# TimoStoff/event_utils

Measured on AMD Instinct MI355X. Metric: Mevents/s (voxel 5-bin 640x480), higher is better.
Workload: dtype f32

## Files before the change

### event_utils_amd/csrc/evk_image2.hip

```cpp
#include "evk_part2.h"
#include "evk_splat.h"

namespace evk {

struct SrcImgF32 {
    static constexpr int G = 4, XYW = 8, TPW = 4;
    const float *x, *y, *w;
    float clipx, clipy;
    float *img;
    int h, wd;
    template <bool NT = false>
    __device__ __forceinline__ void load_xy(int64_t ev0, uint32_t gl, uint32_t *r) const {
        const uint4 a = load_col16<NT>(reinterpret_cast<const float *>(x), ev0, gl), b = load_col16<NT>(reinterpret_cast<const float *>(y), ev0, gl);
        r[0] = a.x, r[1] = a.y, r[2] = a.z, r[3] = a.w, r[4] = b.x, r[5] = b.y, r[6] = b.z, r[7] = b.w;
    }
    template <bool NT = false>
    __device__ __forceinline__ void load_tp(int64_t ev0, uint32_t gl, uint32_t *r) const {
        const uint4 a = load_col16<NT>(w, ev0, gl);
        r[0] = a.x, r[1] = a.y, r[2] = a.z, r[3] = a.w;
    }
    __device__ __forceinline__ int key_of(const uint32_t *r, int e, const TileGridG &g, uint32_t &cell) const {
        const float xf = __uint_as_float(r[e]), yf = __uint_as_float(r[4 + e]);
        const bool keep = !(xf >= clipx) & !(yf >= clipy);
        return nearest_key_cell_int(keep ? (int)xf : 0, keep ? (int)yf : 0, !keep | ((xf == xf) & (yf == yf)), g, cell);
// ... 830 lines not shown
        const int pl = i / dcells;
        __hip_atomic_store(mine + i, lds_cell(pl, i - pl * dcells), __ATOMIC_RELAXED, __HIP_MEMORY_SCOPE_AGENT);
    }
    if (!img_last_part(index, ntiles, it)) return;
    const float *parts = staging + (int64_t)it.first_item * stride;
    flush([&](int pl, int c) {
        float sum = 0.0f;
        for (uint32_t pp = 0; pp < it.nparts; ++pp)
            sum += __hip_atomic_load(parts + (int64_t)pp * stride + pl * dcells + c, __ATOMIC_RELAXED, __HIP_MEMORY_SCOPE_AGENT);
        return sum;
    });
}

static inline int img_window_cells(int tw, int th) { return (tw + 1) * (th + 1); }

static inline bool img_small(int ntiles) {
    return ntiles <= 680 || v2_part_lds(1024, 12, V2_FMT_IMGB, ntiles) > (size_t)V2_LDS_LIMIT;
}
struct ImgCall {
    TileGridG g;
    Part2 q;
    V2Layout L;
    int ntiles;
    bool small;
};
#define IMG_TS_PLANES 6
static int img_setup(ImgCall &ic, int64_t n, int h, int wd, int tile_w, int tile_h, int flags, const void *out, uint32_t *index,
                     void *scratch, int64_t scratch_bytes, uint32_t *host_report, int planes = 2, bool small_only = false) {
    const int known = EVK_VOXEL_OVERWRITE | EVK_VOXEL2_PARTITION_ONLY | EVK_VOXEL2_TILES_ONLY | EVK_VOXEL2_NO_XCD_ORDER |
                      EVK_IMAGE2_NO_FIXED;
    if (make_grid_g(ic.g, h, wd, tile_w, tile_h) != EVK_OK || !out || !index || !scratch || n <= 0 ||
        n > (int64_t)4000000000LL || (flags & ~known))
        return EVK_EINVAL;
    if (host_report && ((uintptr_t)host_report & 7u)) return EVK_EALIGN;
    ic.ntiles = ic.g.tiles_x * ic.g.tiles_y;
    if (ic.ntiles > evk_voxel2_max_tiles() || !evk_voxel2_num_tiles(h, wd, tile_w, tile_h) ||
        (tile_w + 2) * (tile_h + 1) > IMG_WIN_MAX)
        return EVK_EINVAL;
    const bool small = small_only || img_small(ic.ntiles);
    ic.small = small;
    ic.L = v2_layout(ic.ntiles, n, planes, tile_w, tile_h, small);
    if (scratch_bytes < ic.L.total) return EVK_ESCRATCH;
    if (!aligned16(scratch)) return EVK_EALIGN;
    ic.q = v2_geometry(n, ic.ntiles, small);
    return EVK_OK;
}

template <int FMT, typename C>
static void img_partition(const C &c, int64_t n, const ImgCall &ic, uint32_t *index, void *scratch, uint32_t *oob,
                          uint32_t *host_report, uint32_t seq, hipStream_t s, int t_from_events = 0) {
    char *sb = (char *)scratch;
    if constexpr (FMT == V2_FMT_IMGX || FMT == V2_FMT_IMGD) {
        launch_part<1024, 8, FMT>(c, n, ic.g, ic.ntiles, ic.q, 0.0f, 0.0f, 0.0f, t_from_events, sb + ic.L.rec, sb + ic.L.pw,
                                  (uint32_t *)(sb + ic.L.bases), (uint32_t *)(sb + ic.L.table), index, oob, host_report, seq, s);
    } else if (ic.small) {
        launch_part<1024, 8, FMT>(c, n, ic.g, ic.ntiles, ic.q, 0.0f, 0.0f, 0.0f, t_from_events, sb + ic.L.rec, sb + ic.L.pw,
                                  (uint32_t *)(sb + ic.L.bases), (uint32_t *)(sb + ic.L.table), index, oob, host_report, seq, s);
    } else {
        launch_part<1024, 12, FMT>(c, n, ic.g, ic.ntiles, ic.q, 0.0f, 0.0f, 0.0f, t_from_events, sb + ic.L.rec, sb + ic.L.pw,
                                   (uint32_t *)(sb + ic.L.bases), (uint32_t *)(sb + ic.L.table), index, oob, host_report, seq, s);
    }
}

}

using namespace evk;

// ... 194 lines not shown
```

### event_utils_amd/csrc/evk_part2.h

```cpp
#pragma once
#include <cstdio>
#include <cstring>
#include <mutex>
#include <type_traits>

#include "evk_part.h"

namespace evk {

#define V2_HDR 16
#define V2_MAX_TILES 2048
#define V2_TOTALS V2_HDR
#define V2_LIVE_PROGRESS (V2_HDR + V2_MAX_TILES)
#define V2_LIVE_STATUS (V2_LIVE_PROGRESS + 256)
#define V2_PART (V2_LIVE_STATUS + V2_MAX_TILES)
#define V2_COUNTER(T) (V2_PART + (T) + 1)
#define V2_ITEM(T) (V2_PART + 2 * (T) + 1)
#define V2_LB 10
#define EVK_VOXEL2_COUNT (1 << 20)
#define EVK_VOXEL2_COUNT2 (1 << 21)
#define V2_LOCAL_MASK ((1u << V2_LB) - 1u)
#define V2_WIDE (1u << V2_LB)
#define V2_P_MASK (~((2u << V2_LB) - 1u))
__device__ __forceinline__ void lds_barrier() { asm volatile("s_waitcnt lgkmcnt(0)\n\ts_barrier" ::: "memory"); }
// ... 372 lines not shown
                uint32_t word = (d << V2_DELTA_SHIFT) | (code << V2_CODE_SHIFT) | (kl[s2] & V2_LOCAL_MASK);
                if (__any(esc)) {
                    if (esc) {
                        const uint32_t e = atomicAdd(&tmp[67], 1u);
                        wide2[lo + e] = make_uint2(tbits, pb);
                        word = (e << V2_DELTA_SHIFT) | (3u << V2_CODE_SHIFT) | (kl[s2] & V2_LOCAL_MASK);
                        ++nwide;
                    }
                }
                if (live) sorted4[slot_of(s2)] = word;
            }
        }
        lds_barrier();
        if constexpr (EARLY) {
            if (sc == sc_end - 1 && tid == 0 && early_prev == gridDim.x - 1) early_publish();
        }
        if constexpr (LIVE) {
            if (sc > sc0 && tid == 0)
                __hip_atomic_store(live_progress + blockIdx.x, (live_epoch << 8) | (uint32_t)(sc - sc0), __ATOMIC_RELAXED,
                                   __HIP_MEMORY_SCOPE_AGENT);
        }
        EVK_WAIT_VM0();
        kept_prev = kept, lo_prev = lo, sc_prev = sc;
    }
    uint32_t *gidx = index;
    if constexpr (EARLY) {
        if (sc0 >= sc_end && tid == 0) {
            early_prev = __hip_atomic_fetch_add(index + 8, 1u, __ATOMIC_RELAXED, __HIP_MEMORY_SCOPE_AGENT);
            if (early_prev == gridDim.x - 1) early_publish();
        }
    } else {
        if (dropped && oob) atomicAdd(oob, dropped);
    }
    for (int i = tid; i < ntiles; i += THREADS)
        if (tot[i]) __hip_atomic_fetch_add(gidx + V2_TOTALS + i, tot[i], __ATOMIC_RELAXED, __HIP_MEMORY_SCOPE_AGENT);
    {
        uint32_t nw = nwide & 0xFFFFu, nu = nwide >> 16;
#pragma unroll
        for (int off = 32; off >= 1; off >>= 1) nw += __shfl_xor(nw, off, 64), nu += __shfl_xor(nu, off, 64);
        if (lane == 0) {
            if (nw) __hip_atomic_fetch_add(&tmp[66], nw, __ATOMIC_RELAXED, __HIP_MEMORY_SCOPE_WORKGROUP);
            if (nu) __hip_atomic_fetch_add(&tmp[68], nu, __ATOMIC_RELAXED, __HIP_MEMORY_SCOPE_WORKGROUP);
        }
    }
    if (sc0 < sc_end) write_out();
    lds_barrier();
    if (tid == 0) {
        const uint32_t nw = tmp[66], nu = tmp[68];
        if (nw) __hip_atomic_fetch_add(gidx + 3, nw, __ATOMIC_RELAXED, __HIP_MEMORY_SCOPE_AGENT);
        if (nu) __hip_atomic_fetch_add(gidx + 5, nu, __ATOMIC_RELAXED, __HIP_MEMORY_SCOPE_AGENT);
    }
    if constexpr (VOX) {
        if (blockIdx.x == 0 && tid == 0 && n > 0) {
            __hip_atomic_store(gidx + 0, __float_as_uint(c.t1(0)), __ATOMIC_RELAXED, __HIP_MEMORY_SCOPE_AGENT);
            __hip_atomic_store(gidx + 1, __float_as_uint(c.t1(n - 1)), __ATOMIC_RELAXED, __HIP_MEMORY_SCOPE_AGENT);
        }
    }
    EVK_HANDOVER_DRAIN();
    if constexpr (LIVE) {
        if (sc0 < sc_end && tid == 0)
            __hip_atomic_store(live_progress + blockIdx.x, (live_epoch << 8) | (uint32_t)(sc_end - sc0), __ATOMIC_RELAXED,
                               __HIP_MEMORY_SCOPE_AGENT);
    }
    if (tid == 0) {
        const uint32_t prev = __hip_atomic_fetch_add(gidx + 2, 1u, __ATOMIC_RELAXED, __HIP_MEMORY_SCOPE_AGENT);
        is_last = (prev == gridDim.x - 1);
    }
    __syncthreads();
    if (!is_last) return;
    EVK_HANDOVER_ACQUIRE();
    const int per = (ntiles + THREADS - 1) / THREADS;
    const int i0 = tid * per, i1 = (i0 + per < ntiles) ? i0 + per : ntiles;
    uint32_t *part_start = index + V2_PART, *counters = index + V2_COUNTER(ntiles), *item_tile = index + V2_ITEM(ntiles);
    uint32_t tt[PER_MAX];
    uint32_t np = 0;
    uint32_t now5 = 0, prev6 = 0, cnt_oob = 0, now3 = 0, prev0 = 0;
    if (tid == 0) {
        now5 = __hip_atomic_load(gidx + 5, __ATOMIC_RELAXED, __HIP_MEMORY_SCOPE_AGENT);
        prev6 = __hip_atomic_load(gidx + 6, __ATOMIC_RELAXED, __HIP_MEMORY_SCOPE_AGENT);
        if constexpr (!VOX) {
            now3 = __hip_atomic_load(gidx + 3, __ATOMIC_RELAXED, __HIP_MEMORY_SCOPE_AGENT);
            prev0 = __hip_atomic_load(gidx + 0, __ATOMIC_RELAXED, __HIP_MEMORY_SCOPE_AGENT);
        }
        if (!EARLY && host_report && oob) cnt_oob = __hip_atomic_load(oob, __ATOMIC_RELAXED, __HIP_MEMORY_SCOPE_AGENT);
    }
#pragma unroll
    for (int k = 0; k < PER_MAX; ++k) {
        const int i = i0 + k;
        tt[k] = 0;
        if (k < per && i < i1) {
            tt[k] = __hip_atomic_load(gidx + V2_TOTALS + i, __ATOMIC_RELAXED, __HIP_MEMORY_SCOPE_AGENT);
            __hip_atomic_store(gidx + V2_TOTALS + i, 0u, __ATOMIC_RELAXED, __HIP_MEMORY_SCOPE_AGENT);
            np += tt[k] > cap ? (tt[k] + part - 1) / part : 1u;
        }
    }
    uint32_t total_parts;
    uint32_t prun = block_excl_scan<THREADS>(np, tmp, total_parts);
#pragma unroll
    for (int k = 0; k < PER_MAX; ++k) {
        const int i = i0 + k;
        if (k < per && i < i1) {
            const uint32_t parts = tt[k] > cap ? (tt[k] + part - 1) / part : 1u;
            part_start[i] = prun;
            counters[i] = 0;
            for (uint32_t jj = 0; jj < parts; ++jj) item_tile[prun + jj] = (uint32_t)i;
            prun += parts;
        }
    }
    if (tid == 0) {
        part_start[ntiles] = total_parts;
        __hip_atomic_store(gidx + 2, 0u, __ATOMIC_RELAXED, __HIP_MEMORY_SCOPE_AGENT);
        __hip_atomic_store(gidx + 7, now5 != prev6 ? 1u : 0u, __ATOMIC_RELAXED, __HIP_MEMORY_SCOPE_AGENT);
        __hip_atomic_store(gidx + 6, now5, __ATOMIC_RELAXED, __HIP_MEMORY_SCOPE_AGENT);
        if constexpr (!VOX) {
            __hip_atomic_store(gidx + 1, now3 != prev0 ? 1u : 0u, __ATOMIC_RELAXED, __HIP_MEMORY_SCOPE_AGENT);
            __hip_atomic_store(gidx + 0, now3, __ATOMIC_RELAXED, __HIP_MEMORY_SCOPE_AGENT);
        }
        if (!EARLY && host_report) {
            const uint32_t cnt = cnt_oob;
            __hip_atomic_store(reinterpret_cast<unsigned long long *>(host_report),
                               (unsigned long long)seq | ((unsigned long long)cnt << 32), __ATOMIC_RELAXED, __HIP_MEMORY_SCOPE_SYSTEM);
        }
    }
}

struct V2Config {
    int threads, ept;
};
#define V2_GEOMETRIES(X) X(1024, 8) X(1024, 12)
static const V2Config &v2_config(bool share = false, int ntiles = 0) {
    static const V2Config small{1024, 8}, large{1024, 12};
    return (share || ntiles <= 680) ? small : large;
}
#define V2_MIN_SUBCHUNK 8192
#define V2_LDS_LIMIT (160 * 1024 - 512)
static size_t v2_part_lds(int threads, int ept, int rec, int ntiles, bool live = false) {
    return (size_t)threads * ept * v2_fmt_lds_bytes(rec) + 16 + 3 * (size_t)((ntiles + 4) & ~3) * 4 + 72 * 4 + 16 +
           (live ? (size_t)((ntiles + 15) & ~15) * 4 + 16 : 0);
}

static Part2 v2_geometry(int64_t n, int ntiles, bool share = false) {
    const V2Config &c = v2_config(share, ntiles);
    const int64_t smax = (int64_t)c.threads * c.ept;
    int64_t nblk = (n + V2_MIN_SUBCHUNK - 1) / V2_MIN_SUBCHUNK;
    const int64_t maxblk = (int64_t)EVK_NUM_CU * (1024 / c.threads);
    if (nblk > maxblk) nblk = maxblk;
    if (nblk < 1) nblk = 1;
    int64_t per_block = (n + nblk * smax - 1) / (nblk * smax);
    if (per_block < 1) per_block = 1;
    int64_t S = (n + nblk * per_block - 1) / (nblk * per_block);
    S = (S + 3) & ~(int64_t)3;
    if (S < 4) S = 4;
    Part2 q;
    q.S = (int)S, q.per_block = (int)per_block, q.nblk = (int)nblk;
    q.nsc = (int)((n + S - 1) / S);
    if (q.nsc < 1) q.nsc = 1;
// ... 11 lines not shown
}
static int64_t v2_part(int64_t n, int ntiles) {
    const int64_t c = (int64_t)(V2_SPLIT_PART * (double)v2_mean(n, ntiles));
    return c > 8192 ? c : 8192;
}
static int v2_max_items(int64_t n, int ntiles) { return ntiles + (int)(n / v2_part(n, ntiles)) + 1; }

static int v2_rec_bytes(int64_t n, int flags) {
    if (flags & EVK_VOXEL2_REC4) return 4;
    if (flags & EVK_VOXEL2_REC8) return 8;
    return n * 16 > ((int64_t)256 << 20) ? 4 : 8;
}
struct V2Layout {
    int64_t table, bases, rec, pw, staging, total;
};
static V2Layout v2_layout(int ntiles, int64_t n, int planes, int tw, int th, bool share = false) {
    const Part2 q = v2_geometry(n, ntiles, share);
    const int64_t slots = (int64_t)q.nsc * q.S;
    V2Layout L;
    L.table = 0;
    L.bases = al256((int64_t)q.nsc * q.nt_pad * 4);
    L.rec = L.bases + al256((int64_t)q.nsc * 4);
    L.pw = L.rec + al256(slots * 8);
    L.staging = L.pw + al256(slots * 8);
    L.total = L.staging + al256((int64_t)v2_max_items(n, ntiles) * v2_staging_stride((int64_t)planes * tw * th) * 8);
    return L;
}

template <int THREADS, int EPT, int REC, typename C, bool LIVE = false>
static void launch_part(const C &c, int64_t n, const TileGridG &g, int ntiles, const Part2 &q, float t_first, float t_last,
                        float bm1, int t_from_events, void *rec, void *pw, uint32_t *bases, uint32_t *table, uint32_t *index,
                        uint32_t *oob, uint32_t *host_report, uint32_t seq, hipStream_t s, uint32_t *live_progress = nullptr,
                        uint32_t live_epoch = 0) {
    const size_t lds = v2_part_lds(THREADS, EPT, REC, ntiles, LIVE);
    static std::once_flag once[64];
    int dev = 0;
    (void)hipGetDevice(&dev);
    std::call_once(once[dev & 63], [] {
        (void)hipFuncSetAttribute((const void *)k_part_sorted<THREADS, EPT, REC, C, LIVE>, hipFuncAttributeMaxDynamicSharedMemorySize,
                                  160 * 1024 - 256);
    });
    k_part_sorted<THREADS, EPT, REC, C, LIVE><<<q.nblk, THREADS, lds, s>>>(c, n, g, ntiles, q, t_first, t_last, bm1, t_from_events,
                                                                          rec, pw, bases, table, index, (uint32_t)v2_cap(n, ntiles), (uint32_t)v2_part(n, ntiles), oob,
                                                                          host_report, seq, live_progress, live_epoch);
}

}
```

### event_utils_amd/csrc/evk_voxel2.hip

```cpp
#include <atomic>

#include <hip/hip_ext.h>

#include "evk_part2.h"
#include "evk_voxel_live.h"

namespace evk {

__host__ __device__ constexpr int v2_max_chunks(int wg) { return wg == 768 ? 6 : 7; }
__host__ __device__ constexpr int v2_chunk_cap(int wg) { return 64 * v2_max_chunks(wg); }
#define V2_FIXED_ONE 4294967296.0
struct Band {
    int tile_lo, tile_hi, y_lo, rows;
};
template <int WG, int U, bool SPLIT, bool FIXED, int REC>
__global__ void __launch_bounds__(WG, REC == 4 ? 4 : 6) k_voxel_tiles2(const void *__restrict__ rec_, const void *__restrict__ side_,
                                                     const uint32_t *__restrict__ bases,
                                                     const uint32_t *__restrict__ table, uint32_t *__restrict__ index,
                                                     TileGridG g, Part2 q, int B, int flags, float *__restrict__ vox,
                                                     float *__restrict__ staging, Band band, uint32_t *live_status = nullptr,
                                                     uint32_t live_epoch = 0) {
    constexpr int NW = WG / 64, E = REC == 4 ? 3 : 1;
    typedef typename std::conditional<REC == 8, uint4, uint2>::type Pair;
    const float *const pw = static_cast<const float *>(side_);
    const uint2 *const wide2 = static_cast<const uint2 *>(side_);
    const int overwrite = flags & EVK_VOXEL_OVERWRITE;
    constexpr bool split = SPLIT;
    const int NB = split ? 2 * B : B;
    const float bm1 = (float)(B - 1);
    extern __shared__ __attribute__((aligned(16))) acc_t acc[];
    __shared__ uint2 cseg[NW][v2_chunk_cap(WG) + 1];
    __shared__ uint32_t cbase[REC == 4 ? NW : 1][REC == 4 ? v2_chunk_cap(WG) + 1 : 1];
    const int ntiles = g.tiles_x * g.tiles_y;
    const uint32_t *part_start = index + V2_PART, *item_tile = index + V2_ITEM(ntiles);
    const uint32_t nitems_all = part_start[ntiles];
    uint32_t item_lo = 0, nitems = nitems_all;
    if (band.tile_hi > 0) item_lo = part_start[band.tile_lo], nitems = part_start[band.tile_hi] - item_lo;
    if (blockIdx.x >= nitems) return;
    uint32_t item = blockIdx.x;
    if (!(flags & EVK_VOXEL2_NO_XCD_ORDER) && nitems_all == (uint32_t)ntiles) {
        const uint32_t k = blockIdx.x & 7u, j = blockIdx.x >> 3, q8 = nitems >> 3, r8 = nitems & 7u;
        item = k * q8 + (k < r8 ? k : r8) + j;
    }
    item += item_lo;
    const int tw = g.tw, th = g.th, tpix = tw * th;
    const int tpitch = g.pitch, ppix = tpitch * th;
    int tile = (int)item;
    uint32_t first_item = item, nparts = 1u;
    if (nitems_all != (uint32_t)ntiles) {
        tile = (int)item_tile[item];
        first_item = part_start[tile], nparts = part_start[tile + 1] - first_item;
    }
    const uint32_t part_id = item - first_item;
    if (live_status) {
        __shared__ int live_mine;
        if (threadIdx.x == 0) live_mine = v2l_tile_is_mine(live_status + tile, live_epoch) ? 1 : 0;
        __syncthreads();
        if (!live_mine) return;
    }
    const int tx0 = (tile % g.tiles_x) * tw, ty0 = (tile / g.tiles_x) * th;
    constexpr double G_ONE = 2147483648.0;
    __shared__ uint32_t poison[(1 << V2_LB) / 32];
    constexpr bool COUNTING = !SPLIT;
    const bool unit = COUNTING && (flags & EVK_VOXEL2_COUNT) && index[7] == 0u;
    const bool unit2 = COUNTING && !unit && (flags & EVK_VOXEL2_COUNT2) && index[7] == 0u;
    int *const s0 = reinterpret_cast<int *>(acc + (B + 1) * ppix);
    unsigned long long *const gq = reinterpret_cast<unsigned long long *>(acc);
    if (threadIdx.x < NW) {
        cseg[threadIdx.x][v2_chunk_cap(WG)] = make_uint2(0u, 0u);
        if constexpr (REC == 4) cbase[threadIdx.x][v2_chunk_cap(WG)] = 0u;
    }
    if (unit) {
        for (int i = threadIdx.x; i < (B + 1) * ppix; i += WG) acc[i] = 0.0;
        for (int i = threadIdx.x; i < B * ppix; i += WG) s0[i] = 0;
        if (threadIdx.x < (1 << V2_LB) / 32) poison[threadIdx.x] = 0u;
    } else {
        for (int i = threadIdx.x; i < NB * ppix; i += WG) acc[i] = 0.0;
        if ((FIXED || unit2) && threadIdx.x < (1 << V2_LB) / 32) poison[threadIdx.x] = 0u;
    }
    const int sc_lo = (int)(((int64_t)q.nsc * part_id) / nparts), sc_hi = (int)(((int64_t)q.nsc * (part_id + 1)) / nparts);
    const uint32_t *col = table + tile;
    const int lane = threadIdx.x & 63, wave = threadIdx.x >> 6, sub = lane & 3, grp = lane >> 2;
    auto add = [&](acc_t *a, float v) {
        if constexpr (FIXED) {
            const double sc = (double)v * V2_FIXED_ONE;
            if (!(fabs(sc) < 4.0e18)) {
                __hip_atomic_fetch_add(index + 4, 1u, __ATOMIC_RELAXED, __HIP_MEMORY_SCOPE_AGENT);
                return;
            }
            __hip_atomic_fetch_add(reinterpret_cast<unsigned long long *>(a), (unsigned long long)__double2ll_rn(sc), __ATOMIC_RELAXED,
                                   __HIP_MEMORY_SCOPE_WORKGROUP);
        } else {
            lds_add(a, v);
        }
    };
    auto bins_general = [&](acc_t *base, int local, float tn, float p) {
        if (tn != tn) {
            if constexpr (FIXED) {
                __hip_atomic_fetch_or(poison + (local >> 5), 1u << (local & 31), __ATOMIC_RELAXED, __HIP_MEMORY_SCOPE_WORKGROUP);
                return;
            }
            for (int b = 0; b < B; ++b) add(base + b * ppix + local, tn * p);
            return;
        }
        if (!(fabsf(p) <= 3.0e38f)) {
            for (int b = 0; b < B; ++b) add(base + b * ppix + local, p * fmaxf(0.0f, 1.0f - fabsf(tn - (float)b)));
            return;
        }
        const float fl = floorf(tn);
        const int b0 = (int)fmaxf(fminf(fl, (float)(B + 1)), -2.0f);
#pragma unroll
        for (int k = 0; k < 2; ++k) {
            const int b = b0 + k;
            if (b < 0 || b >= B) continue;
            const float val = p * fmaxf(0.0f, 1.0f - fabsf(tn - (float)b));
// ... 185 lines not shown
        Pair va[U], vb[U];
        meta(0u, ca, ba);
        fire(ca, va);
        meta(step, cb, bbv);
        for (uint32_t j0 = 0; j0 < total; j0 += 2u * step) {
            fire(cb, vb);
            meta(j0 + 2u * step, cn, bn);
            eat(ca, ba, va);
            fire(cn, va);
#pragma unroll
            for (int u = 0; u < U; ++u) ca[u] = cn[u], ba[u] = bn[u];
            meta(j0 + 3u * step, cn, bn);
            eat(cb, bbv, vb);
#pragma unroll
            for (int u = 0; u < U; ++u) cb[u] = cn[u], bbv[u] = bn[u];
        }
    };
    auto stream_segment = [&](auto unit_tag, const uint32_t b2, const uint32_t e3, const uint32_t b2b) {
        for (uint32_t p2 = b2 + 2u * lane; p2 < e3; p2 += 512u) {
            Pair v[4];
#pragma unroll
            for (int u = 0; u < 4; ++u) {
                const uint32_t pu = p2 + 128u * u;
                v[u] = load_pair(pu < e3 ? pu : p2);
            }
#pragma unroll
            for (int u = 0; u < 4; ++u) {
                const uint32_t pu = p2 + 128u * u;
                if (pu < e3) pair(unit_tag, v[u], b2b, pu, e3);
            }
        }
    };
    auto wave_scan = [&](uint32_t v) { return wave_incl_scan_u32(v); };
    const int range = sc_hi - sc_lo;
    auto batches = [&](auto unit_tag) {
    if constexpr (E > 1) {
        const int nbatch = (range + WG * E - 1) / (WG * E);
        const int bsz = nbatch ? ((range + nbatch - 1) / nbatch + NW - 1) / NW * NW : NW;
        auto fetch = [&](int base, uint32_t(&en)[E], uint32_t(&bn)[E]) {
#pragma unroll
            for (int e = 0; e < E; ++e) {
                const int idx = (e * 64 + lane) * NW + wave, my = base + idx;
                const bool have = idx < bsz && my < sc_hi;
                en[e] = have ? col[(int64_t)my * q.nt_pad] : 0u;
                bn[e] = 0u;
                if constexpr (REC == 4) bn[e] = have ? bases[my] : 0u;
            }
        };
        uint32_t ent[E], bb[E];
        fetch(sc_lo, ent, bb);
        __syncthreads();
        for (int base = sc_lo; base < sc_hi; base += bsz) {
            uint32_t sum = 0, longs = 0, packed = 0;
            auto mych_of = [&](int e) { return (packed >> (4 * e)) & 15u; };
#pragma unroll
            for (int e = 0; e < E; ++e) {
                const uint32_t cnt = ent[e] >> 16;
                const uint32_t nch = (cnt + 7u) >> 3;
                const bool is_long = nch > (uint32_t)v2_max_chunks(WG);
                packed |= (is_long ? 0u : nch) << (4 * e);
                sum += is_long ? 0u : nch;
                longs |= is_long ? (1u << e) : 0u;
            }
            const uint32_t incl_all = wave_scan(sum);
            const bool fits = wave_bcast_u32(incl_all, 63) <= (uint32_t)v2_chunk_cap(WG);
            const int npass = fits ? 1 : E;
            for (int pass = 0; pass < npass; ++pass) {
                uint32_t mine = sum, incl = incl_all;
                if (pass > 0) fetch(base, ent, bb);
                if (!fits) {
                    mine = 0;
#pragma unroll
                    for (int e = 0; e < E; ++e) mine = e == pass ? mych_of(e) : mine;
                    incl = wave_scan(mine);
                }
                const uint32_t total = wave_bcast_u32(incl, 63);
                uint32_t w = incl - mine;
#pragma unroll
                for (int e = 0; e < E; ++e) {
                    if (!fits && e != pass) continue;
                    const uint32_t start = ent[e] & 0xFFFFu, cnt = ent[e] >> 16;
                    const uint32_t rb = (uint32_t)(base + (e * 64 + lane) * NW + wave) * (uint32_t)q.S, p0 = rb + start, e0 = p0 + cnt;
                    const uint32_t mc = mych_of(e);
// ... 2 lines not shown
                        if constexpr (REC == 4) cbase[wave][w + k] = bb[e];
                    }
                    w += mc;
                }
                rounds(unit_tag, total);
            }
            fetch(base + bsz, ent, bb);
            uint32_t nlong = 0;
            if (__ballot(longs != 0u)) {
                uint32_t ent2[E], bb2[E];
                fetch(base, ent2, bb2);
#pragma unroll
                for (int e = 0; e < E; ++e) {
                    const bool il = (longs >> e) & 1u;
                    const uint64_t m = __ballot(il);
                    if (il) {
                        const uint32_t st = ent2[e] & 0xFFFFu, cn = ent2[e] >> 16;
                        const uint32_t rb = (uint32_t)(base + (e * 64 + lane) * NW + wave) * (uint32_t)q.S;
                        const uint32_t at = nlong + (uint32_t)__builtin_popcountll(m & ((1ull << lane) - 1ull));
                        cseg[wave][at] = make_uint2(rb + st, rb + st + cn);
                        if constexpr (REC == 4) cbase[wave][at] = bb2[e];
                    }
                    nlong += (uint32_t)__builtin_popcountll(m);
                }
            }
            for (uint32_t i = 0; i < nlong; ++i) {
                const uint2 sg = cseg[wave][i];
                uint32_t b2b = 0u;
                if constexpr (REC == 4) b2b = cbase[wave][i];
                stream_segment(unit_tag, sg.x, sg.y, b2b);
            }
        }
    } else {
        const int nbatch = (range + WG - 1) / WG;
        const int bsz = nbatch ? ((range + nbatch - 1) / nbatch + NW - 1) / NW * NW : NW;
        const int slot = lane * NW + wave;
        uint32_t ent_next = 0, bb_next = 0;
        {
            const int my = sc_lo + slot;
            if (slot < bsz && my < sc_hi) {
                ent_next = col[(int64_t)my * q.nt_pad];
                if constexpr (REC == 4) bb_next = bases[my];
            }
        }
        for (int base = sc_lo; base < sc_hi; base += bsz) {
            const uint32_t ent = ent_next, bb = bb_next;
            {
                const int my = base + bsz + slot;
                const bool have = slot < bsz && my < sc_hi;
                ent_next = have ? col[(int64_t)my * q.nt_pad] : 0u;
                if constexpr (REC == 4) bb_next = have ? bases[my] : 0u;
            }
            const uint32_t start = ent & 0xFFFFu, cnt = ent >> 16;
            const uint32_t nch = (cnt + 7u) >> 3;
            const uint32_t incl_full = wave_scan(nch);
            const uint32_t total_full = wave_bcast_u32(incl_full, 63);
            uint32_t npass = (total_full + (uint32_t)v2_chunk_cap(WG) - 1u) / (uint32_t)v2_chunk_cap(WG);
            npass = npass < 1u ? 1u : (npass > 4u ? 4u : npass);
            __syncthreads();
            for (uint32_t pass = 0; pass < npass; ++pass) {
                const bool mine = npass == 1u || ((uint32_t)lane * npass) / 64u == pass;
                uint32_t mych = mine ? nch : 0u, incl = incl_full;
                bool is_long = false;
                if (npass > 1u) {
                    incl = wave_scan(mych);
                    if (wave_bcast_u32(incl, 63) > (uint32_t)v2_chunk_cap(WG)) {
                        is_long = mine && nch > (uint32_t)v2_max_chunks(WG);
                        mych = (mine && !is_long) ? nch : 0u;
                        incl = wave_scan(mych);
                    }
                }
                const uint32_t total = wave_bcast_u32(incl, 63), excl = incl - mych;
                {
                    const uint32_t rb = (uint32_t)(base + slot) * (uint32_t)q.S, p0 = rb + start, e0 = p0 + cnt;
                    for (uint32_t k = 0; k < mych; ++k) {
                        cseg[wave][excl + k] = make_uint2(p0 + 8u * k, e0);
                        if constexpr (REC == 4) cbase[wave][excl + k] = bb;
// ... 59 lines not shown
            return (float)((double)__builtin_bit_cast(long long, a) * (1.0 / V2_FIXED_ONE));
        }
        return (float)a;
    };
    if (nparts == 1) {
        flush(lds_cell);
        return;
    }
    const int cells = NB * tpix;
    const int64_t stride = v2_staging_stride(cells);
    const bool exactq = unit || unit2 || FIXED;
    const double qscale = (unit || unit2) ? 1.0 / G_ONE : 1.0 / V2_FIXED_ONE;
    auto lds_cell_q = [&](int c) -> long long {
        int b, row, col;
        split_cell(c, b, row, col);
        const int l = row * tpitch + col;
        if (unit) {
            if ((poison[l >> 5] >> (l & 31)) & 1u) return (long long)0x8000000000000000ull;
            return ((long long)s0[b * ppix + l] << 31) - (long long)gq[(b + 1) * ppix + l] + (long long)gq[b * ppix + l];
        }
        if ((FIXED || unit2) && ((poison[l >> 5] >> (l & 31)) & 1u)) return (long long)0x8000000000000000ull;
        return __builtin_bit_cast(long long, acc[b * ppix + l]);
    };
    float *mine = staging + 2 * (int64_t)item * stride;
    if (exactq) {
        unsigned long long *mq = reinterpret_cast<unsigned long long *>(mine);
        for (int c = threadIdx.x; c < cells; c += WG)
            __hip_atomic_store(mq + c, (unsigned long long)lds_cell_q(c), __ATOMIC_RELAXED, __HIP_MEMORY_SCOPE_AGENT);
    } else {
        for (int c = threadIdx.x; c < cells; c += WG)
            __hip_atomic_store(mine + c, lds_cell(c), __ATOMIC_RELAXED, __HIP_MEMORY_SCOPE_AGENT);
    }
    EVK_HANDOVER_DRAIN();
    __shared__ int is_last;
    if (threadIdx.x == 0) {
        uint32_t *counter = index + V2_COUNTER(ntiles) + tile;
        const uint32_t prev = __hip_atomic_fetch_add(counter, 1u, __ATOMIC_RELAXED, __HIP_MEMORY_SCOPE_AGENT);
        is_last = (prev == nparts - 1);
        if (is_last) __hip_atomic_store(counter, 0u, __ATOMIC_RELAXED, __HIP_MEMORY_SCOPE_AGENT);
    }
    __syncthreads();
    if (!is_last) return;
    EVK_HANDOVER_ACQUIRE();
    const float *parts = staging + 2 * (int64_t)first_item * stride;
    if (exactq) {
        const unsigned long long *pq = reinterpret_cast<const unsigned long long *>(parts);
        flush([&](int c) {
            long long sum = 0;
            bool nan = false;
            for (uint32_t p = 0; p < nparts; ++p) {
                const long long v = (long long)__hip_atomic_load(pq + (int64_t)p * stride + c, __ATOMIC_RELAXED, __HIP_MEMORY_SCOPE_AGENT);
                nan |= v == (long long)0x8000000000000000ull;
                sum += v;
            }
            return nan ? __uint_as_float(0x7FC00000u) : (float)((double)sum * qscale);
        });
        return;
    }
    flush([&](int c) {
        float sum = 0.0f;
        for (uint32_t p = 0; p < nparts; ++p)
            sum += __hip_atomic_load(parts + 2 * (int64_t)p * stride + c, __ATOMIC_RELAXED, __HIP_MEMORY_SCOPE_AGENT);
        return sum;
    });
}

}
// ... 76 lines not shown
    std::call_once(once[dev & 63], [dev] {
        ev[dev & 63] = nullptr;
        if (hipEventCreateWithFlags(&ev[dev & 63], hipEventDisableTiming) != hipSuccess) ev[dev & 63] = nullptr;
    });
    return ev[dev & 63];
}
static uint32_t v2_live_epoch() {
    static std::atomic<uint32_t> counter{0};
    uint32_t e;
    do e = (counter.fetch_add(1, std::memory_order_relaxed) + 1u) & V2L_EPOCH_MASK; while (e == 0u);
    return e;
}
#define V2L_STATIC_LDS (V2L_NW * V2L_CAP * 8 + 2 * ((1 << V2_LB) / 32) * 4 + 64)
static bool v2_live_fits(const TileGridG &g, int ntiles, const Part2 &q, int64_t n, int B, int recb, const V2Config &cfg) {
    const size_t acc = (size_t)2 * B * g.pitch * g.th * 8;
    return recb == 8 && cfg.threads == 1024 && cfg.ept == 8 && ntiles <= 2 * EVK_NUM_CU && q.nblk <= V2L_PROGRESS_WORDS &&
           q.per_block >= 2 && q.per_block <= 255 && n < ((int64_t)1 << 28) && (int64_t)q.nsc * q.S * 8 < ((int64_t)1 << 32) &&
           acc + V2L_STATIC_LDS <= (size_t)V2L_LDS_REQUEST &&
           v2_part_lds(1024, 8, 8, ntiles, true) + 256 + V2L_LDS_REQUEST <= (size_t)160 * 1024;
}

template <typename C>
static int voxel2(const C &c, int64_t n, int h, int wd, int tile_w, int tile_h, float t_first, float t_last, int B,
                  int flags, float *vox, uint32_t *index, void *scratch, int64_t scratch_bytes, uint32_t *oob,
                  uint32_t *host_report, uint32_t seq, void *stream, const Band &band = Band{0, 0, 0, 0}) {
    TileGridG g;
    const int known = EVK_VOXEL_OVERWRITE | EVK_VOXEL_SPLIT_POLARITY | EVK_VOXEL_T_FROM_EVENTS | EVK_VOXEL2_PARTITION_ONLY |
                      EVK_VOXEL2_TILES_ONLY | EVK_VOXEL2_NO_XCD_ORDER | EVK_VOXEL2_SHARE_CU | EVK_VOXEL_DETERMINISTIC |
                      EVK_VOXEL2_REC4 | EVK_VOXEL2_REC8 | EVK_VOXEL2_NO_COUNT | EVK_VOXEL2_WG512 | EVK_VOXEL2_LIVE | EVK_VOXEL2_NO_COUNT2;
    if (make_grid_g(g, h, wd, tile_w, tile_h) != EVK_OK || B <= 0 || !vox || !index || !scratch || n <= 0 ||
        n > (int64_t)4000000000LL || (flags & ~known))
        return EVK_EINVAL;
    if (host_report && ((uintptr_t)host_report & 7u)) return EVK_EALIGN;
    const int ntiles = g.tiles_x * g.tiles_y;
    if (ntiles > evk_voxel2_max_tiles() || !evk_voxel2_num_tiles(h, wd, tile_w, tile_h)) return EVK_EINVAL;
    const int planes = (flags & EVK_VOXEL_SPLIT_POLARITY) ? 2 * B : B;
    const size_t lds_acc = (size_t)planes * sizeof(acc_t) * g.pitch * g.th;
    if (v2_tiles_lds(g, planes) > (size_t)V2_TILES_LDS_LIMIT) return EVK_EINVAL;
    const bool share = flags & EVK_VOXEL2_SHARE_CU;
    const V2Layout L = v2_layout(ntiles, n, planes, tile_w, tile_h, share);
    if (scratch_bytes < L.total) return EVK_ESCRATCH;
    if (!aligned16(scratch)) return EVK_EALIGN;
    const Part2 q = v2_geometry(n, ntiles, share);
    char *sb = (char *)scratch;
    uint32_t *table = (uint32_t *)(sb + L.table), *bases = (uint32_t *)(sb + L.bases);
    void *rec = sb + L.rec, *pw = sb + L.pw;
    float *staging = (float *)(sb + L.staging);
    hipStream_t s = (hipStream_t)stream;
    const V2Config &cfg = v2_config(share, ntiles);
    const float bm1 = (float)(B - 1);
    const int tfe = (flags & EVK_VOXEL_T_FROM_EVENTS) ? 1 : 0;
    const int recb = v2_rec_bytes(n, flags);
    bool live = false;
    hipStream_t s2 = nullptr;
    hipEvent_t live_done = nullptr;
    uint32_t epoch = 0;
    if constexpr (std::is_same<C, SrcF32>::value) {
        if ((flags & EVK_VOXEL2_LIVE) && band.tile_hi == 0 &&
            !(flags & (EVK_VOXEL2_PARTITION_ONLY | EVK_VOXEL2_TILES_ONLY | EVK_VOXEL_SPLIT_POLARITY | EVK_VOXEL2_SHARE_CU |
                       EVK_VOXEL2_NO_COUNT)) &&
            v2_live_fits(g, ntiles, q, n, B, recb, cfg)) {
            hipStreamCaptureStatus cap = hipStreamCaptureStatusNone;
            if (hipStreamIsCapturing(s, &cap) == hipSuccess && cap == hipStreamCaptureStatusNone && (s2 = v2_live_stream()) != nullptr)
                live = true, epoch = v2_live_epoch();
            else
                (void)hipGetLastError();
// ... 126 lines not shown
```

Baseline: 146,200.

## Pack tile totals into 64-bit atomics and skip last-block scan when no tile splits

Partition blocks now add per-tile totals two at a time with 64-bit atomics, and each block detects whether its addition crossed the split cap. These cut flags, plus nonunit and wide flags, are folded into the block-completion ticket, so the last block skips the full prefix/split scan when no tile needs splitting. The tile kernel reads a compact header (index[7], index[9]) and issues its first table fetch before zeroing LDS and resolving items, which overlaps global latency with setup. This adds alignment requirements on index and limits the ticket to 256 workgroups per field.

```diff
diff --git a/event_utils_amd/csrc/evk_image2.hip b/event_utils_amd/csrc/evk_image2.hip
--- a/event_utils_amd/csrc/evk_image2.hip
+++ b/event_utils_amd/csrc/evk_image2.hip
@@ -886,7 +886,7 @@
     if (make_grid_g(ic.g, h, wd, tile_w, tile_h) != EVK_OK || !out || !index || !scratch || n <= 0 ||
         n > (int64_t)4000000000LL || (flags & ~known))
         return EVK_EINVAL;
-    if (host_report && ((uintptr_t)host_report & 7u)) return EVK_EALIGN;
+    if ((host_report && ((uintptr_t)host_report & 7u)) || ((uintptr_t)index & 7u)) return EVK_EALIGN;
     ic.ntiles = ic.g.tiles_x * ic.g.tiles_y;
     if (ic.ntiles > evk_voxel2_max_tiles() || !evk_voxel2_num_tiles(h, wd, tile_w, tile_h) ||
         (tile_w + 2) * (tile_h + 1) > IMG_WIN_MAX)
diff --git a/event_utils_amd/csrc/evk_part2.h b/event_utils_amd/csrc/evk_part2.h
--- a/event_utils_amd/csrc/evk_part2.h
+++ b/event_utils_amd/csrc/evk_part2.h
@@ -428,8 +428,17 @@
     } else {
         if (dropped && oob) atomicAdd(oob, dropped);
     }
-    for (int i = tid; i < ntiles; i += THREADS)
-        if (tot[i]) __hip_atomic_fetch_add(gidx + V2_TOTALS + i, tot[i], __ATOMIC_RELAXED, __HIP_MEMORY_SCOPE_AGENT);
+    static_assert(V2_MAX_TILES / 2 <= THREADS, "one pair of tiles per thread");
+    static_assert((V2_TOTALS & 1) == 0, "the packed totals are 8-byte aligned");
+    unsigned long long *const gtot2 = reinterpret_cast<unsigned long long *>(gidx + V2_TOTALS);
+    uint32_t mine_lo = 0, mine_hi = 0;
+    unsigned long long old2 = 0;
+    if (2 * tid < ntiles) {
+        mine_lo = tot[2 * tid], mine_hi = 2 * tid + 1 < ntiles ? tot[2 * tid + 1] : 0u;
+        if (mine_lo | mine_hi)
+            old2 = __hip_atomic_fetch_add(gtot2 + tid, (unsigned long long)mine_lo | ((unsigned long long)mine_hi << 32), __ATOMIC_RELAXED,
+                                          __HIP_MEMORY_SCOPE_AGENT);
+    }
     {
         uint32_t nw = nwide & 0xFFFFu, nu = nwide >> 16;
 #pragma unroll
@@ -441,16 +450,22 @@
     }
     if (sc0 < sc_end) write_out();
     lds_barrier();
+    uint32_t my_nw = 0, my_nu = 0;
     if (tid == 0) {
-        const uint32_t nw = tmp[66], nu = tmp[68];
-        if (nw) __hip_atomic_fetch_add(gidx + 3, nw, __ATOMIC_RELAXED, __HIP_MEMORY_SCOPE_AGENT);
-        if (nu) __hip_atomic_fetch_add(gidx + 5, nu, __ATOMIC_RELAXED, __HIP_MEMORY_SCOPE_AGENT);
+        my_nw = tmp[66], my_nu = tmp[68];
+        if (my_nw) __hip_atomic_fetch_add(gidx + 3, my_nw, __ATOMIC_RELAXED, __HIP_MEMORY_SCOPE_AGENT);
+        if (my_nu) __hip_atomic_fetch_add(gidx + 5, my_nu, __ATOMIC_RELAXED, __HIP_MEMORY_SCOPE_AGENT);
     }
     if constexpr (VOX) {
         if (blockIdx.x == 0 && tid == 0 && n > 0) {
             __hip_atomic_store(gidx + 0, __float_as_uint(c.t1(0)), __ATOMIC_RELAXED, __HIP_MEMORY_SCOPE_AGENT);
             __hip_atomic_store(gidx + 1, __float_as_uint(c.t1(n - 1)), __ATOMIC_RELAXED, __HIP_MEMORY_SCOPE_AGENT);
         }
+    }
+    asm volatile("s_waitcnt vmcnt(0)" ::: "memory");
+    {
+        const uint32_t old_lo = (uint32_t)old2, old_hi = (uint32_t)(old2 >> 32);
+        if ((old_lo <= cap && old_lo + mine_lo > cap) || (old_hi <= cap && old_hi + mine_hi > cap)) tmp[70] = 1u;
     }
     EVK_HANDOVER_DRAIN();
     if constexpr (LIVE) {
@@ -458,28 +473,41 @@
             __hip_atomic_store(live_progress + blockIdx.x, (live_epoch << 8) | (uint32_t)(sc_end - sc0), __ATOMIC_RELAXED,
                                __HIP_MEMORY_SCOPE_AGENT);
     }
+    __shared__ uint32_t ticket_prev;
     if (tid == 0) {
-        const uint32_t prev = __hip_atomic_fetch_add(gidx + 2, 1u, __ATOMIC_RELAXED, __HIP_MEMORY_SCOPE_AGENT);
-        is_last = (prev == gridDim.x - 1);
+        const uint32_t mine = 1u | (tmp[70] ? 1u << 8 : 0u) | (my_nu ? 1u << 16 : 0u) | (my_nw ? 1u << 24 : 0u);
+        const uint32_t prev = __hip_atomic_fetch_add(gidx + 2, mine, __ATOMIC_RELAXED, __HIP_MEMORY_SCOPE_AGENT);
+        is_last = ((prev & 0xFFu) == gridDim.x - 1);
+        const uint32_t all = prev | mine;
+        ticket_prev = ((all >> 8) & 0xFFu ? 1u : 0u) | ((all >> 16) & 0xFFu ? 2u : 0u) | (all >> 24 ? 4u : 0u);
     }
     __syncthreads();
     if (!is_last) return;
     EVK_HANDOVER_ACQUIRE();
+    uint32_t *part_start = index + V2_PART, *counters = index + V2_COUNTER(ntiles), *item_tile = index + V2_ITEM(ntiles);
+    const uint32_t seen = ticket_prev;
+    const bool any_cut = seen & 1u, any_nu = seen & 2u, any_nw = seen & 4u;
+    auto header = [&](uint32_t items) {
+        part_start[ntiles] = items;
+        __hip_atomic_store(gidx + 2, 0u, __ATOMIC_RELAXED, __HIP_MEMORY_SCOPE_AGENT);
+        __hip_atomic_store(gidx + 7, any_nu ? 1u : 0u, __ATOMIC_RELAXED, __HIP_MEMORY_SCOPE_AGENT);
+        __hip_atomic_store(gidx + 9, items, __ATOMIC_RELAXED, __HIP_MEMORY_SCOPE_AGENT);
+        if constexpr (!VOX) __hip_atomic_store(gidx + 1, any_nw ? 1u : 0u, __ATOMIC_RELAXED, __HIP_MEMORY_SCOPE_AGENT);
+        if (!EARLY && host_report) {
+            const uint32_t cnt = oob ? __hip_atomic_load(oob, __ATOMIC_RELAXED, __HIP_MEMORY_SCOPE_AGENT) : 0u;
+            __hip_atomic_store(reinterpret_cast<unsigned long long *>(host_report),
+                               (unsigned long long)seq | ((unsigned long long)cnt << 32), __ATOMIC_RELAXED, __HIP_MEMORY_SCOPE_SYSTEM);
+        }
+    };
+    if (!any_cut) {
+        if (2 * tid < ntiles) __hip_atomic_store(gtot2 + tid, 0ull, __ATOMIC_RELAXED, __HIP_MEMORY_SCOPE_AGENT);
+        if (tid == 0) header((uint32_t)ntiles);
+        return;
+    }
     const int per = (ntiles + THREADS - 1) / THREADS;
     const int i0 = tid * per, i1 = (i0 + per < ntiles) ? i0 + per : ntiles;
-    uint32_t *part_start = index + V2_PART, *counters = index + V2_COUNTER(ntiles), *item_tile = index + V2_ITEM(ntiles);
     uint32_t tt[PER_MAX];
     uint32_t np = 0;
-    uint32_t now5 = 0, prev6 = 0, cnt_oob = 0, now3 = 0, prev0 = 0;
-    if (tid == 0) {
-        now5 = __hip_atomic_load(gidx + 5, __ATOMIC_RELAXED, __HIP_MEMORY_SCOPE_AGENT);
-        prev6 = __hip_atomic_load(gidx + 6, __ATOMIC_RELAXED, __HIP_MEMORY_SCOPE_AGENT);
-        if constexpr (!VOX) {
-            now3 = __hip_atomic_load(gidx + 3, __ATOMIC_RELAXED, __HIP_MEMORY_SCOPE_AGENT);
-            prev0 = __hip_atomic_load(gidx + 0, __ATOMIC_RELAXED, __HIP_MEMORY_SCOPE_AGENT);
-        }
-        if (!EARLY && host_report && oob) cnt_oob = __hip_atomic_load(oob, __ATOMIC_RELAXED, __HIP_MEMORY_SCOPE_AGENT);
-    }
 #pragma unroll
     for (int k = 0; k < PER_MAX; ++k) {
         const int i = i0 + k;
@@ -503,21 +531,7 @@
             prun += parts;
         }
     }
-    if (tid == 0) {
-        part_start[ntiles] = total_parts;
-        __hip_atomic_store(gidx + 2, 0u, __ATOMIC_RELAXED, __HIP_MEMORY_SCOPE_AGENT);
-        __hip_atomic_store(gidx + 7, now5 != prev6 ? 1u : 0u, __ATOMIC_RELAXED, __HIP_MEMORY_SCOPE_AGENT);
-        __hip_atomic_store(gidx + 6, now5, __ATOMIC_RELAXED, __HIP_MEMORY_SCOPE_AGENT);
-        if constexpr (!VOX) {
-            __hip_atomic_store(gidx + 1, now3 != prev0 ? 1u : 0u, __ATOMIC_RELAXED, __HIP_MEMORY_SCOPE_AGENT);
-            __hip_atomic_store(gidx + 0, now3, __ATOMIC_RELAXED, __HIP_MEMORY_SCOPE_AGENT);
-        }
-        if (!EARLY && host_report) {
-            const uint32_t cnt = cnt_oob;
-            __hip_atomic_store(reinterpret_cast<unsigned long long *>(host_report),
-                               (unsigned long long)seq | ((unsigned long long)cnt << 32), __ATOMIC_RELAXED, __HIP_MEMORY_SCOPE_SYSTEM);
-        }
-    }
+    if (tid == 0) header(total_parts);
 }
 
 struct V2Config {
@@ -595,6 +609,7 @@
                         float bm1, int t_from_events, void *rec, void *pw, uint32_t *bases, uint32_t *table, uint32_t *index,
                         uint32_t *oob, uint32_t *host_report, uint32_t seq, hipStream_t s, uint32_t *live_progress = nullptr,
                         uint32_t live_epoch = 0) {
+    static_assert(EVK_NUM_CU * (1024 / THREADS) <= 256, "the ticket counts at most 256 workgroups per field");
     const size_t lds = v2_part_lds(THREADS, EPT, REC, ntiles, LIVE);
     static std::once_flag once[64];
     int dev = 0;
diff --git a/event_utils_amd/csrc/evk_voxel2.hip b/event_utils_amd/csrc/evk_voxel2.hip
--- a/event_utils_amd/csrc/evk_voxel2.hip
+++ b/event_utils_amd/csrc/evk_voxel2.hip
@@ -33,54 +33,83 @@
     __shared__ uint32_t cbase[REC == 4 ? NW : 1][REC == 4 ? v2_chunk_cap(WG) + 1 : 1];
     const int ntiles = g.tiles_x * g.tiles_y;
     const uint32_t *part_start = index + V2_PART, *item_tile = index + V2_ITEM(ntiles);
-    const uint32_t nitems_all = part_start[ntiles];
-    uint32_t item_lo = 0, nitems = nitems_all;
-    if (band.tile_hi > 0) item_lo = part_start[band.tile_lo], nitems = part_start[band.tile_hi] - item_lo;
-    if (blockIdx.x >= nitems) return;
-    uint32_t item = blockIdx.x;
-    if (!(flags & EVK_VOXEL2_NO_XCD_ORDER) && nitems_all == (uint32_t)ntiles) {
-        const uint32_t k = blockIdx.x & 7u, j = blockIdx.x >> 3, q8 = nitems >> 3, r8 = nitems & 7u;
-        item = k * q8 + (k < r8 ? k : r8) + j;
-    }
-    item += item_lo;
+    __shared__ uint32_t poison[(1 << V2_LB) / 32];
+    __shared__ int live_mine, is_last;
+    constexpr bool COUNTING = !SPLIT;
+    const uint32_t hdr_nonunit = index[7], nitems_all = index[9];
+    const uint32_t W = band.tile_hi > 0 ? (uint32_t)(band.tile_hi - band.tile_lo) : (uint32_t)ntiles;
+    const uint32_t tile_lo = band.tile_hi > 0 ? (uint32_t)band.tile_lo : 0u;
+    const bool surplus = blockIdx.x >= W;
+    if (surplus && nitems_all == (uint32_t)ntiles) return;
     const int tw = g.tw, th = g.th, tpix = tw * th;
     const int tpitch = g.pitch, ppix = tpitch * th;
+    int *const s0 = reinterpret_cast<int *>(acc + (B + 1) * ppix);
+    unsigned long long *const gq = reinterpret_cast<unsigned long long *>(acc);
+    const int lane = threadIdx.x & 63, wave = threadIdx.x >> 6, sub = lane & 3, grp = lane >> 2;
+    if (threadIdx.x < NW) {
+        cseg[threadIdx.x][v2_chunk_cap(WG)] = make_uint2(0u, 0u);
+        if constexpr (REC == 4) cbase[threadIdx.x][v2_chunk_cap(WG)] = 0u;
+    }
+    uint32_t item = tile_lo;
+    if (!surplus) {
+        item = blockIdx.x;
+        if (!(flags & EVK_VOXEL2_NO_XCD_ORDER)) {
+            const uint32_t k = blockIdx.x & 7u, j = blockIdx.x >> 3, q8 = W >> 3, r8 = W & 7u;
+            item = k * q8 + (k < r8 ? k : r8) + j;
+        }
+        item += tile_lo;
+    }
     int tile = (int)item;
-    uint32_t first_item = item, nparts = 1u;
+    uint32_t first_item = item, nparts = 1u, part_id = 0u;
+    int sc_lo = 0, sc_hi = q.nsc, range, nbatch, bsz;
+    const uint32_t *col;
+    auto batching = [&]() {
+        col = table + tile;
+        range = sc_hi - sc_lo;
+        nbatch = (range + WG * E - 1) / (WG * E);
+        bsz = nbatch ? ((range + nbatch - 1) / nbatch + NW - 1) / NW * NW : NW;
+    };
+    batching();
+    auto fetch = [&](int base, uint32_t(&en)[E], uint32_t(&bn)[E]) {
+#pragma unroll
+        for (int e = 0; e < E; ++e) {
+            const int idx = (e * 64 + lane) * NW + wave, my = base + idx;
+            const bool have = idx < bsz && my < sc_hi;
+            en[e] = have ? col[(int64_t)my * q.nt_pad] : 0u;
+            bn[e] = 0u;
+            if constexpr (REC == 4) bn[e] = have ? bases[my] : 0u;
+        }
+    };
+    uint32_t ent0[E] = {}, bb0[E] = {};
+    if (!surplus) fetch(sc_lo, ent0, bb0);
+    if (COUNTING && (flags & EVK_VOXEL2_COUNT)) {
+        for (int i = threadIdx.x; i < (B + 1) * ppix; i += WG) acc[i] = 0.0;
+        for (int i = threadIdx.x; i < B * ppix; i += WG) s0[i] = 0;
+    } else {
+        for (int i = threadIdx.x; i < NB * ppix; i += WG) acc[i] = 0.0;
+    }
+    if (threadIdx.x < (1 << V2_LB) / 32) poison[threadIdx.x] = 0u;
+    const bool unit = COUNTING && (flags & EVK_VOXEL2_COUNT) && hdr_nonunit == 0u;
+    const bool unit2 = COUNTING && !unit && (flags & EVK_VOXEL2_COUNT2) && hdr_nonunit == 0u;
     if (nitems_all != (uint32_t)ntiles) {
+        uint32_t item_lo = 0u, nitems = nitems_all;
+        if (band.tile_hi > 0) item_lo = part_start[band.tile_lo], nitems = part_start[band.tile_hi] - item_lo;
+        if (blockIdx.x >= nitems) return;
+        item = item_lo + blockIdx.x;
         tile = (int)item_tile[item];
         first_item = part_start[tile], nparts = part_start[tile + 1] - first_item;
-    }
-    const uint32_t part_id = item - first_item;
+        part_id = item - first_item;
+        sc_lo = (int)(((int64_t)q.nsc * part_id) / nparts), sc_hi = (int)(((int64_t)q.nsc * (part_id + 1)) / nparts);
+        batching();
+        fetch(sc_lo, ent0, bb0);
+    }
     if (live_status) {
-        __shared__ int live_mine;
         if (threadIdx.x == 0) live_mine = v2l_tile_is_mine(live_status + tile, live_epoch) ? 1 : 0;
         __syncthreads();
         if (!live_mine) return;
     }
     const int tx0 = (tile % g.tiles_x) * tw, ty0 = (tile / g.tiles_x) * th;
     constexpr double G_ONE = 2147483648.0;
-    __shared__ uint32_t poison[(1 << V2_LB) / 32];
-    constexpr bool COUNTING = !SPLIT;
-    const bool unit = COUNTING && (flags & EVK_VOXEL2_COUNT) && index[7] == 0u;
-    const bool unit2 = COUNTING && !unit && (flags & EVK_VOXEL2_COUNT2) && index[7] == 0u;
-    int *const s0 = reinterpret_cast<int *>(acc + (B + 1) * ppix);
-    unsigned long long *const gq = reinterpret_cast<unsigned long long *>(acc);
-    if (threadIdx.x < NW) {
-        cseg[threadIdx.x][v2_chunk_cap(WG)] = make_uint2(0u, 0u);
-        if constexpr (REC == 4) cbase[threadIdx.x][v2_chunk_cap(WG)] = 0u;
-    }
-    if (unit) {
-        for (int i = threadIdx.x; i < (B + 1) * ppix; i += WG) acc[i] = 0.0;
-        for (int i = threadIdx.x; i < B * ppix; i += WG) s0[i] = 0;
-        if (threadIdx.x < (1 << V2_LB) / 32) poison[threadIdx.x] = 0u;
-    } else {
-        for (int i = threadIdx.x; i < NB * ppix; i += WG) acc[i] = 0.0;
-        if ((FIXED || unit2) && threadIdx.x < (1 << V2_LB) / 32) poison[threadIdx.x] = 0u;
-    }
-    const int sc_lo = (int)(((int64_t)q.nsc * part_id) / nparts), sc_hi = (int)(((int64_t)q.nsc * (part_id + 1)) / nparts);
-    const uint32_t *col = table + tile;
-    const int lane = threadIdx.x & 63, wave = threadIdx.x >> 6, sub = lane & 3, grp = lane >> 2;
     auto add = [&](acc_t *a, float v) {
         if constexpr (FIXED) {
             const double sc = (double)v * V2_FIXED_ONE;
@@ -332,23 +361,11 @@
         }
     };
     auto wave_scan = [&](uint32_t v) { return wave_incl_scan_u32(v); };
-    const int range = sc_hi - sc_lo;
     auto batches = [&](auto unit_tag) {
     if constexpr (E > 1) {
-        const int nbatch = (range + WG * E - 1) / (WG * E);
-        const int bsz = nbatch ? ((range + nbatch - 1) / nbatch + NW - 1) / NW * NW : NW;
-        auto fetch = [&](int base, uint32_t(&en)[E], uint32_t(&bn)[E]) {
-#pragma unroll
-            for (int e = 0; e < E; ++e) {
-                const int idx = (e * 64 + lane) * NW + wave, my = base + idx;
-                const bool have = idx < bsz && my < sc_hi;
-                en[e] = have ? col[(int64_t)my * q.nt_pad] : 0u;
-                bn[e] = 0u;
-                if constexpr (REC == 4) bn[e] = have ? bases[my] : 0u;
-            }
-        };
         uint32_t ent[E], bb[E];
-        fetch(sc_lo, ent, bb);
+#pragma unroll
+        for (int e = 0; e < E; ++e) ent[e] = ent0[e], bb[e] = bb0[e];
         __syncthreads();
         for (int base = sc_lo; base < sc_hi; base += bsz) {
             uint32_t sum = 0, longs = 0, packed = 0;
@@ -417,17 +434,8 @@
             }
         }
     } else {
-        const int nbatch = (range + WG - 1) / WG;
-        const int bsz = nbatch ? ((range + nbatch - 1) / nbatch + NW - 1) / NW * NW : NW;
         const int slot = lane * NW + wave;
-        uint32_t ent_next = 0, bb_next = 0;
-        {
-            const int my = sc_lo + slot;
-            if (slot < bsz && my < sc_hi) {
-                ent_next = col[(int64_t)my * q.nt_pad];
-                if constexpr (REC == 4) bb_next = bases[my];
-            }
-        }
+        uint32_t ent_next = ent0[0], bb_next = bb0[0];
         for (int base = sc_lo; base < sc_hi; base += bsz) {
             const uint32_t ent = ent_next, bb = bb_next;
             {
@@ -553,7 +561,6 @@
             __hip_atomic_store(mine + c, lds_cell(c), __ATOMIC_RELAXED, __HIP_MEMORY_SCOPE_AGENT);
     }
     EVK_HANDOVER_DRAIN();
-    __shared__ int is_last;
     if (threadIdx.x == 0) {
         uint32_t *counter = index + V2_COUNTER(ntiles) + tile;
         const uint32_t prev = __hip_atomic_fetch_add(counter, 1u, __ATOMIC_RELAXED, __HIP_MEMORY_SCOPE_AGENT);
@@ -696,6 +703,7 @@
         n > (int64_t)4000000000LL || (flags & ~known))
         return EVK_EINVAL;
     if (host_report && ((uintptr_t)host_report & 7u)) return EVK_EALIGN;
+    if ((uintptr_t)index & 7u) return EVK_EALIGN;
     const int ntiles = g.tiles_x * g.tiles_y;
     if (ntiles > evk_voxel2_max_tiles() || !evk_voxel2_num_tiles(h, wd, tile_w, tile_h)) return EVK_EINVAL;
     const int planes = (flags & EVK_VOXEL_SPLIT_POLARITY) ? 2 * B : B;
```

Measured after the change: 145,200. About the same (-0.6%).
